# bssrdf/CUDA-Winograd

Hardware: AMD Instinct MI355X
Metric: effective_tflops_conv3x3_256_bn_relu_14x14_N128_fp32 (higher is better)
Workload: dtype f32

## Files before the change

### cuda-winograd_amd/csrc/wino_f2_fused_kernel.h

```cpp
#pragma once
#include "wino_common.h"

#include <type_traits>

namespace wino {
namespace fused {

constexpr int TB = 64;
constexpr int KB = 64;
constexpr int BC = 8;
constexpr int NTHREADS = 512;
constexpr int RAW_BYTES = TB * 16 * BC * 4;
constexpr int U_BYTES = 16 * KB * BC * 4;
constexpr int N_RSTAGE = 2, N_USTAGE = 3;
constexpr int LDS_BYTES = N_RSTAGE * RAW_BYTES + N_USTAGE * U_BYTES;
constexpr int U_CHUNK_FLOATS = 16 * KB * BC;
constexpr int PF = 2;
constexpr int SLAB_BYTES = TB * 4 * KB * 4;
constexpr int DMA0 = 4;

__device__ __forceinline__ void wait_lds(int n) {
  switch (n) {
    case 0: __builtin_amdgcn_s_waitcnt(0xC07F); break;
    case 1: __builtin_amdgcn_s_waitcnt(0xC17F); break;
    case 2: __builtin_amdgcn_s_waitcnt(0xC27F); break;
    case 3: __builtin_amdgcn_s_waitcnt(0xC37F); break;
    case 4: __builtin_amdgcn_s_waitcnt(0xC47F); break;
    case 5: __builtin_amdgcn_s_waitcnt(0xC57F); break;
    case 6: __builtin_amdgcn_s_waitcnt(0xC67F); break;
    case 7: __builtin_amdgcn_s_waitcnt(0xC77F); break;
    case 8: __builtin_amdgcn_s_waitcnt(0xC87F); break;
    case 9: __builtin_amdgcn_s_waitcnt(0xC97F); break;
    case 10: __builtin_amdgcn_s_waitcnt(0xCA7F); break;
    case 11: __builtin_amdgcn_s_waitcnt(0xCB7F); break;
    case 12: __builtin_amdgcn_s_waitcnt(0xCC7F); break;
    default: __builtin_amdgcn_s_waitcnt(0xCF7F); break;
  }
}
constexpr int lds_nr(int q) { return q < 6 ? 2 : 0; }
constexpr int lds_n(int q) { return 2 + lds_nr(q); }
constexpr int lds_wait_count(int e) {
  int after = 15;
  if (e >= PF) {
    after = lds_nr(e - PF);
    for (int q = e - PF + 1; q <= e; q++) after += lds_n(q);
  }
  return after > 15 ? 15 : after;
}

__device__ __forceinline__ f32x2 lds_read2(int addr) {
  return *(const __attribute__((address_space(3))) f32x2*)(size_t)(unsigned)addr;
}
struct TileCoord {
  int n, ty, tx;
};
__device__ __forceinline__ TileCoord decode_tile(int g) {
  TileCoord t;
  t.n = g / WINO_TILES;
  const int rem = g - t.n * WINO_TILES;
  t.ty = rem / 7;
  t.tx = rem - t.ty * 7;
  return t;
}

struct Geo {
  int Hp, Wp;
  unsigned tiles, tiles_x;
  FastDiv d_tiles, d_tx;
};
template <bool GEN>
__device__ __forceinline__ TileCoord decode_tile_g(int g, const Geo& geo) {
  if (!GEN) return decode_tile(g);
  TileCoord t;
  t.n = (int)fastdiv((unsigned)g, geo.d_tiles);
  const unsigned rem = (unsigned)g - (unsigned)t.n * geo.tiles;
  t.ty = (int)fastdiv(rem, geo.d_tx);
  t.tx = (int)(rem - (unsigned)t.ty * geo.tiles_x);
  return t;
}

__host__ __device__ inline unsigned sk_start(unsigned l, unsigned q, unsigned rem, unsigned G) {
  return l * q + l * rem / G;
}

__host__ __device__ inline int tail_range_of(int j, int P, int inv, int copies) {
  const int r = j / copies, b = j - r * copies;
  return (inv * r) % P + P * b;
}
__device__ __forceinline__ int tail_range_of_fast(int j, int P, int inv, int copies, FastDiv d_P, FastDiv d_copies) {
  const int r = (int)fastdiv((unsigned)j, d_copies), b = j - r * copies;
  const int ir = inv * r;
  return ir - (int)fastdiv((unsigned)ir, d_P) * P + P * b;
}

struct FusedParams {
  const float* in;
  const float* Uq;
  int N, C, K, relu, nTB;
  int ndp;
  unsigned sk_q, sk_rem;
  int kp;
  int Gp;
  int ph_P, ph_inv, ph_copies;
  FastDiv d_kp, d_P, d_copies;
  Geo geo;
  const float* bnBias;
  const float* bnScale;
  float* out;
  float* slabs;
  unsigned* tickets;
  unsigned* err;
  unsigned long long* dbg;
};
struct FusedResParams : FusedParams {
  const float* res;
};
template <bool RES>
using FusedArgs = std::conditional_t<RES, FusedResParams, FusedParams>;
constexpr int EPI_PLAIN = 0, EPI_RES = 1, EPI_POOL = 2;

inline void fused_work_layout(FusedParams& p, long long items, int G) {
  const int nchunks = p.C / BC, kblk = p.K / KB;
  const int kp = kblk <= 1 || (G % kblk) != 0 ? 1 : kblk;
  const long long Tg = (items % G) * nchunks / kp, Gp = G / kp, q = Tg / Gp, rem = Tg % Gp;
  p.ndp = (int)(items / G);
  p.sk_q = (unsigned)q;
  p.sk_rem = (unsigned)rem;
  p.kp = kp;
  p.Gp = (int)Gp;
  p.ph_P = 1, p.ph_inv = 0, p.ph_copies = (int)Gp;
  if (rem == 0 && q > 0) {
    long long a = q % nchunks, b = nchunks;
    while (a) { const long long t = b % a; b = a; a = t; }
    const long long g = b, P = nchunks / g;
    if (P > 1 && Gp % P == 0) {
      const long long qq = (q / g) % P;
      for (long long x = 1; x < P; x++)
        if ((qq * x) % P == 1) { p.ph_P = (int)P; p.ph_inv = (int)x; p.ph_copies = (int)(Gp / P); break; }
    }
  }
  p.d_kp = make_fastdiv((unsigned)kp);
  p.d_P = make_fastdiv((unsigned)p.ph_P);
  p.d_copies = make_fastdiv((unsigned)p.ph_copies);
}

__device__ unsigned long long wino_clk_slot_3x3[4];

template <int ABLATE, bool GEN = false, bool TAIL = true, int EPI = EPI_PLAIN>
__global__ void __launch_bounds__(NTHREADS, 2)
wino_f2_fused_kernel(const FusedArgs<EPI == EPI_RES> prm) {
  static_assert(EPI == EPI_PLAIN || EPI == EPI_RES || EPI == EPI_POOL, "epilogue form");
  constexpr bool RES = EPI == EPI_RES, POOL = EPI == EPI_POOL;
  extern __shared__ __attribute__((aligned(16))) char smem[];
  const float* in = prm.in;
  const float* Uq = prm.Uq;
  asm volatile("" : "+s"(in), "+s"(Uq));
  const int N = prm.N, C = prm.C, K = prm.K;
  const unsigned sk_q = prm.sk_q, sk_rem = prm.sk_rem;
  const int ndp = prm.ndp;

  const int KBLK = K >> 6;
  const int nchunks = C / BC;
  const int G = gridDim.x;
  const int lg = (int)(blockIdx.x & 7) * (G >> 3) + ((int)(blockIdx.x & 7) < (G & 7) ? (int)(blockIdx.x & 7) : (G & 7)) +
                 (int)(blockIdx.x >> 3);
  if (ABLATE & PROBE_TIMELINE) {
    if (threadIdx.x == 0) {
      prm.dbg[(size_t)lg * TL_WORDS + TL_ENTRY] = __builtin_amdgcn_s_memrealtime();
      prm.dbg[(size_t)lg * TL_WORDS + TL3_ENTRY_CYC] = __builtin_amdgcn_s_memtime();
    }
  }
  if (ABLATE == PROBE_OFF && blockIdx.x == 0 && threadIdx.x == 0) {
    wino_clk_slot_3x3[0] = __builtin_amdgcn_s_memtime();
    wino_clk_slot_3x3[1] = __builtin_amdgcn_s_memrealtime();
  }
  auto clk_exit = [&]() {
    if (ABLATE == PROBE_OFF && blockIdx.x == 0 && threadIdx.x == 0) {
      wino_clk_slot_3x3[2] = __builtin_amdgcn_s_memtime();
      wino_clk_slot_3x3[3] = __builtin_amdgcn_s_memrealtime();
    }
  };
  const int tail_item0 = ndp * G;
  const int kpg = prm.kp, Gp = prm.Gp;
  const int lpos = __builtin_amdgcn_readfirstlane((int)fastdiv((unsigned)lg, prm.d_kp)), grp = lg - lpos * kpg;
  const int lp = __builtin_amdgcn_readfirstlane(tail_range_of_fast(lpos, prm.ph_P, prm.ph_inv, prm.ph_copies, prm.d_P, prm.d_copies));
  const unsigned t_begin = __builtin_amdgcn_readfirstlane(sk_start(lp, sk_q, sk_rem, Gp));
  const int Lt = (int)(__builtin_amdgcn_readfirstlane(sk_start(lp + 1, sk_q, sk_rem, Gp)) - t_begin);
  const int L = Lt + ndp * nchunks;

  auto ring_pass = [&]() {
    if (ABLATE & PROBE_NO_STORE) return;
    const unsigned Hi = GEN ? (unsigned)prm.geo.Hp : (unsigned)WINO_HW, Wi = GEN ? (unsigned)prm.geo.Wp : (unsigned)WINO_HW;
    const unsigned Hp = POOL ? (Hi - 2u) / 2u + 2u : Hi, Wp = POOL ? (Wi - 2u) / 2u + 2u : Wi;
    const unsigned rpx = 2u * Wp + 2u * (Hp - 2u);
    const unsigned upp = (unsigned)K >> 2;
    const unsigned long long U = (unsigned long long)N * rpx * upp;
    const unsigned u_begin = (unsigned)(U * (unsigned)lg / (unsigned)G);
    const unsigned u_end = (unsigned)(U * ((unsigned)lg + 1u) / (unsigned)G);
    const auto rsrc_ring = make_rsrc(prm.out, (unsigned)((size_t)N * Hp * Wp * K * sizeof(float)));
    const f32x4 zero4 = {0.f, 0.f, 0.f, 0.f};
    for (unsigned u = u_begin + threadIdx.x; u < u_end; u += NTHREADS) {
      const unsigned pid = u / upp, unit = u - pid * upp;
      const unsigned n = pid / rpx, q = pid - n * rpx;
      const unsigned y = q < Wp ? 0u : q < 2 * Wp ? Hp - 1 : q < 2 * Wp + Hp - 2 ? q - 2 * Wp + 1 : q - 2 * Wp - (Hp - 2) + 1;
      const unsigned x = q < Wp ? q : q < 2 * Wp ? q - Wp : q < 2 * Wp + Hp - 2 ? 0u : Wp - 1;
      buf_store16(zero4, rsrc_ring, (((n * Hp + y) * Wp + x) * (unsigned)K + unit * 4u) * (unsigned)sizeof(float), 0);
    }
  };
  if (L <= 0) {
    ring_pass();
    clk_exit();
    return;
  }

  const int tid = threadIdx.x;
  const int lane = tid & 63;
  const int w = __builtin_amdgcn_readfirstlane(tid >> 6);
  const int wt = w >> 1;
  const int ph = w & 1;

  const unsigned u_off = lane * 16;
  const unsigned u_chunk_stride = (unsigned)(KBLK * U_CHUNK_FLOATS * sizeof(float));
  const auto rsrc_in = make_rsrc(in, (unsigned)((size_t)N * (GEN ? prm.geo.Hp * prm.geo.Wp : WINO_HW * WINO_HW) * C * sizeof(float)));
  const auto rsrc_u = make_rsrc(Uq, (unsigned)((size_t)16 * C * K * sizeof(float)));

  const int t16 = lane & 15, h = lane >> 4;
  const int lds0 = (int)(unsigned)(size_t)(__attribute__((address_space(3))) char*)smem;
  const int a_base = lds0 + (wt * 16 + t16) * 512 + ((h ^ (((t16 >> 3) & 1) << 1)) << 3);
  const int a_sw = t16 & 7;
  int a_adr[3][4];
#pragma unroll
  for (int k = 0; k < 3; k++) {
    const int row = ph ? (k == 0 ? 2 : k == 1 ? 1 : 3) : (k == 0 ? 0 : k == 1 ? 2 : 1);
#pragma unroll
    for (int j = 0; j < 4; j++) {
      const int px = 4 * row + j;
      a_adr[k][j] = a_base + (((px & 7) ^ a_sw) << 5) + ((px >> 3) << 8);
    }
  }
  int b_base[4];
#pragma unroll
  for (int cb = 0; cb < 4; cb++) {
    const int kl = (cb ^ (2 * ph)) * 16 + t16;
    b_base[cb] = lds0 + N_RSTAGE * RAW_BYTES + ph * (8 * 2048) + kl * 32 + ((h ^ (((kl >> 3) & 1) << 1)) << 3);
  }
  asm volatile("" : "+v"(b_base[1]), "+v"(b_base[2]), "+v"(b_base[3]));

  typedef f32x2 P2;
  auto sub2 = [](const P2& a, const P2& b) { return a - b; };
  auto add2 = [](const P2& a, const P2& b) { return a + b; };
  const float s2f = ph ? -1.f : 1.f;
  const P2 s2 = {s2f, s2f};
  auto tmp_col = [&](P2* tmp, const P2* d, int j) {
    tmp[0 * 4 + j] = sub2(d[0 * 4 + j], d[1 * 4 + j]);
    tmp[1 * 4 + j] = d[1 * 4 + j] + s2 * d[2 * 4 + j];
  };
  auto v_point = [&](P2* v, const P2* tmp, int e) {
    const int i = e >> 2, j = e & 3;
    if (j == 0) v[e] = sub2(tmp[i * 4 + 0], tmp[i * 4 + 2]);
    if (j == 1) v[e] = add2(tmp[i * 4 + 1], tmp[i * 4 + 2]);
    if (j == 2) v[e] = sub2(tmp[i * 4 + 2], tmp[i * 4 + 1]);
    if (j == 3) v[e] = sub2(tmp[i * 4 + 1], tmp[i * 4 + 3]);
  };

  unsigned long long st_wait = 0, st_comp = 0, st_epi = 0, st_prev = 0;
  unsigned long long st_ph[4] = {0, 0, 0, 0};
  auto stamp = [&]() -> unsigned long long {
    unsigned long long t;
    __builtin_amdgcn_sched_barrier(0);
    asm volatile("s_memtime %0\n\ts_waitcnt lgkmcnt(0)" : "=s"(t)::"memory");
    __builtin_amdgcn_sched_barrier(0);
    return t;
  };

  typedef const __attribute__((address_space(4))) FusedParams* KernargPtr;
  auto kernarg = []() {
    KernargPtr kp = (KernargPtr)__builtin_amdgcn_kernarg_segment_ptr();
    asm volatile("" : "+s"(kp));
    return kp;
  };
  auto load_geo = [](KernargPtr kp) {
    Geo g;
    g.Hp = kp->geo.Hp; g.Wp = kp->geo.Wp; g.tiles = kp->geo.tiles; g.tiles_x = kp->geo.tiles_x;
    g.d_tiles.m = kp->geo.d_tiles.m; g.d_tiles.l = kp->geo.d_tiles.l;
    g.d_tx.m = kp->geo.d_tx.m; g.d_tx.l = kp->geo.d_tx.l;
    return g;
  };

  unsigned raw_off[4];
  unsigned d_soff_raw = 0;
  unsigned d_soff_u = 0;
  int d_item, d_chunk, d_tail, d_tb = -1;
  auto dma_set_item = [&](int item) {
    const int tb = item / KBLK, kb = item - tb * KBLK;
    d_item = item;
    if (tb != d_tb) {
      d_tb = tb;
      KernargPtr kp = kernarg();
      const Geo geo = load_geo(kp);
      const int Wp = GEN ? geo.Wp : WINO_HW, Hp = GEN ? geo.Hp : WINO_HW;
      const int C = kp->C, totalTiles = kp->N * (GEN ? (int)geo.tiles : WINO_TILES);
      const int up = lane & 31;
      const int pxp = up >> 1, halfp = up & 1;
#pragma unroll
      for (int j = 0; j < 4; j++) {
        const int tl = 16 * j + 2 * w + (lane >> 5);
        const int px = pxp ^ (tl & 7);
        const int half = halfp ^ ((tl >> 3) & 1);
        int g = tb * TB + tl;
        g = g < totalTiles ? g : totalTiles - 1;
        const TileCoord tc = decode_tile_g<GEN>(g, geo);
        const int y = 2 * tc.ty + (px >> 2), x = 2 * tc.tx + (px & 3);
        raw_off[j] = (unsigned)((((size_t)(tc.n * Hp + y) * Wp + x) * C + half * 4) * sizeof(float));
      }
    }
    d_soff_raw = __builtin_amdgcn_readfirstlane((unsigned)(d_chunk * (BC * sizeof(float))));
    d_soff_u = __builtin_amdgcn_readfirstlane((unsigned)((kb * U_CHUNK_FLOATS + w * 256) * sizeof(float)) + d_chunk * u_chunk_stride);
    asm volatile("" : "+s"(d_soff_raw), "+s"(d_soff_u));
  };
  auto pin_dma_state = [&]() {
    d_item = __builtin_amdgcn_readfirstlane(d_item);
    d_chunk = __builtin_amdgcn_readfirstlane(d_chunk);
    d_tail = __builtin_amdgcn_readfirstlane(d_tail);
    d_tb = __builtin_amdgcn_readfirstlane(d_tb);
    asm volatile("" : "+s"(d_item), "+s"(d_chunk), "+s"(d_tail), "+s"(d_tb));
  };
  auto dma_advance = [&]() {
    if (d_tail > 0 && --d_tail == 0) {
      d_chunk = 0;
      dma_set_item(lg);
    } else if (++d_chunk == nchunks) {
      d_chunk = 0;
      dma_set_item(d_tail > 0 ? d_item + kernarg()->kp : d_item + G);
    } else {
      d_soff_raw += (unsigned)(BC * sizeof(float));
      d_soff_u += u_chunk_stride;
      asm volatile("" : "+s"(d_soff_raw), "+s"(d_soff_u));
    }
    pin_dma_state();
  };
  auto issue_raw1 = [&](int rstage, int j) {
    if (ABLATE & PROBE_NO_DMA_A) return;
    dma16_buf(rsrc_in, raw_off[j], d_soff_raw, smem + rstage * RAW_BYTES + (8 * j + w) * 1024);
  };
  auto issue_u1 = [&](int ustage, int j) {
    if (ABLATE & PROBE_NO_DMA_B) return;
    dma16_buf(rsrc_u, u_off, d_soff_u + j * 8192,
              smem + N_RSTAGE * RAW_BYTES + ustage * U_BYTES + (8 * j + w) * 1024);
  };

  int c_tail_vg = Lt;
  int c_item_vg = __builtin_amdgcn_readfirstlane(Lt > 0 ? tail_item0 + (int)(t_begin / (unsigned)nchunks) * kpg + grp : lg);
  int c_chunk = __builtin_amdgcn_readfirstlane(Lt > 0 ? (int)(t_begin % (unsigned)nchunks) : 0);
  int seg_kind_vg = 0;
  int pend_vg = -1;
  asm volatile("" : "+v"(pend_vg));

  f32x4 acc[8][4];
#pragma unroll
  for (int e = 0; e < 8; e++)
#pragma unroll
    for (int cb = 0; cb < 4; cb++) acc[e][cb] = (f32x4){0.f, 0.f, 0.f, 0.f};
  P2 v[8];
  f32x2 bfn[PF][2];

  d_chunk = c_chunk;
  d_tail = Lt;
  dma_set_item(c_item_vg);
  asm volatile("" : "+v"(c_item_vg));
#pragma unroll
  for (int j = 0; j < 4; j++) issue_raw1(0, j);
#pragma unroll
  for (int j = 0; j < 4; j++) issue_u1(0, j);
  if ((ABLATE & PROBE_TIMELINE) && tid == 0) prm.dbg[(size_t)lg * TL_WORDS + TL3_STAGE_REQ] = __builtin_amdgcn_s_memrealtime();
  if (L > 1) dma_advance();
  ring_pass();
  if (!(ABLATE & PROBE_NO_SYNC)) {
    wait_vmem_all();
    __syncthreads();
  }
  if ((ABLATE & PROBE_TIMELINE) && tid == 0) prm.dbg[(size_t)lg * TL_WORDS + TL3_STAGE_IN] = __builtin_amdgcn_s_memrealtime();
  if (L > 1) {
#pragma unroll
    for (int j = 0; j < 4; j++) issue_raw1(1, j);
#pragma unroll
    for (int j = 0; j < 4; j++) issue_u1(1, j);
    if (L > 2) dma_advance();
  }
  {
    P2 d[12];
#pragma unroll
    for (int k = 0; k < 3; k++)
#pragma unroll
      for (int j = 0; j < 4; j++) d[k * 4 + j] = lds_read2(a_adr[k][j]);
    P2 tmp[8];
#pragma unroll
    for (int j = 0; j < 4; j++) tmp_col(tmp, d, j);
#pragma unroll
    for (int e = 0; e < 8; e++) v_point(v, tmp, e);
#pragma unroll
    for (int e = 0; e < PF; e++) {
      bfn[e][0] = lds_read2(b_base[2 * (e & 1) + 0] + (e >> 1) * 2048);
      bfn[e][1] = lds_read2(b_base[2 * (e & 1) + 1] + (e >> 1) * 2048);
    }
  }
  if (ABLATE & PROBE_TIMELINE) {
    if (tid == 0) prm.dbg[(size_t)lg * TL_WORDS + TL_FIRST] = __builtin_amdgcn_s_memrealtime();
  }
  if (ABLATE & PROBE_CLOCK) {
    if (tid == 0) {
      prm.dbg[(size_t)lg * CLK_WORDS + CLK_BEGIN_CYC] = __builtin_amdgcn_s_memtime();
      prm.dbg[(size_t)lg * CLK_WORDS + CLK_BEGIN_RT] = __builtin_amdgcn_s_memrealtime();
    }
  }

  int ub_cur[4], ub_nxt[4];
#pragma unroll
  for (int cb = 0; cb < 4; cb++) {
    ub_cur[cb] = b_base[cb];
    ub_nxt[cb] = b_base[cb] + U_BYTES;
  }
  auto body = [&](auto par_c, int it, int rs_dma, int us_dma) {
    constexpr int ROFF = decltype(par_c)::value ? 0 : RAW_BYTES;
    if (ABLATE & PROBE_PHASES) { const unsigned long long t = stamp(); if (it) st_comp += t - st_prev; st_prev = t; }
    if (!(ABLATE & PROBE_NO_SYNC)) {
      wait_vmem_all();
      __syncthreads();
    }
    if (ABLATE & PROBE_PHASES) { const unsigned long long t = stamp(); st_wait += t - st_prev; st_prev = t; }
    const int (&ucur)[4] = decltype(par_c)::value ? ub_nxt : ub_cur;
    const int (&unxt)[4] = decltype(par_c)::value ? ub_cur : ub_nxt;
    auto bread = [&](const int (&base)[4], int s2_, int c) {
      return lds_read2(base[2 * (s2_ & 1) + c] + (s2_ >> 1) * 2048);
    };

    f32x2 bf[16][2];
#pragma unroll
    for (int e = 0; e < PF; e++) { bf[e][0] = bfn[e][0]; bf[e][1] = bfn[e][1]; }
    P2 d[12], tmp[8];
    __builtin_amdgcn_sched_barrier(0);
#pragma unroll
    for (int e = 0; e < 16; e++) {
      const int pt = e >> 1, cbp = e & 1;
      if (ABLATE & PROBE_NO_B_READS) {
        const f32x2 fake = {v[(e + 3) & 7].x, v[(e + 5) & 7].y};
        if (e + PF < 16) { bf[e + PF][0] = fake; bf[e + PF][1] = fake; }
        else { bfn[e + PF - 16][0] = fake; bfn[e + PF - 16][1] = fake; }
      } else if (e + PF < 16) {
        bf[e + PF][0] = bread(ucur, e + PF, 0);
        bf[e + PF][1] = bread(ucur, e + PF, 1);
      } else {
        bfn[e + PF - 16][0] = bread(unxt, e + PF - 16, 0);
        bfn[e + PF - 16][1] = bread(unxt, e + PF - 16, 1);
      }
      if (e >= DMA0 && e < DMA0 + 4) {
        issue_raw1(rs_dma, e - DMA0);
      } else if (e >= DMA0 + 4 && e < DMA0 + 8) {
        issue_u1(us_dma, e - DMA0 - 4);
      }
      if (e < 6 && !(ABLATE & PROBE_NO_A_PATH)) {
        const int q0 = 2 * e, q1 = 2 * e + 1;
        d[(q0 % 3) * 4 + q0 / 3] = lds_read2(a_adr[q0 % 3][q0 / 3] + ROFF);
        d[(q1 % 3) * 4 + q1 / 3] = lds_read2(a_adr[q1 % 3][q1 / 3] + ROFF);
      }
      __builtin_amdgcn_sched_barrier(0);
      if (!(ABLATE & (PROBE_NO_A_PATH | PROBE_NO_B_READS))) wait_lds(lds_wait_count(e));
      __builtin_amdgcn_sched_barrier(0);
      if (e >= 3 && e <= 7 && e != 5 && !(ABLATE & PROBE_NO_A_PATH) && !(ABLATE & PROBE_NO_BTDB)) tmp_col(tmp, d, e == 3 ? 0 : e == 4 ? 1 : e == 6 ? 2 : 3);
      if ((ABLATE & PROBE_NO_BTDB) && e == 7) {
#pragma unroll
        for (int i = 0; i < 12; i++) asm volatile("" :: "v"(d[i]));
      }
      const P2 a = v[pt];
      const f32x2 b0 = bf[e][0], b1 = bf[e][1];
      if (ABLATE & PROBE_NO_MFMA) {
        asm volatile("" ::"v"(a.x), "v"(a.y), "v"(b0.x), "v"(b0.y), "v"(b1.x), "v"(b1.y));
      } else {
        asm volatile("v_mfma_f32_16x16x4_f32 %0, %1, %2, %0" : "+v"(acc[pt][2 * cbp + 0]) : "v"(a.x), "v"(b0.x));
        asm volatile("v_mfma_f32_16x16x4_f32 %0, %1, %2, %0" : "+v"(acc[pt][2 * cbp + 1]) : "v"(a.x), "v"(b1.x));
        asm volatile("v_mfma_f32_16x16x4_f32 %0, %1, %2, %0" : "+v"(acc[pt][2 * cbp + 0]) : "v"(a.y), "v"(b0.y));
        asm volatile("v_mfma_f32_16x16x4_f32 %0, %1, %2, %0" : "+v"(acc[pt][2 * cbp + 1]) : "v"(a.y), "v"(b1.y));
      }
      if ((ABLATE & PROBE_NO_VPOINT) && !(ABLATE & PROBE_NO_BTDB) && e == 9) {
#pragma unroll
        for (int i = 0; i < 8; i++) asm volatile("" :: "v"(tmp[i]));
      }
      if (!(ABLATE & PROBE_NO_A_PATH) && !(ABLATE & (PROBE_NO_VPOINT | PROBE_NO_BTDB))) {
        if (e >= 9 && e < 15) v_point(v, tmp, e - 9);
        if (e == 15) {
          v_point(v, tmp, 6);
          v_point(v, tmp, 7);
        }
      }
      __builtin_amdgcn_sched_barrier(0);
    }
  };

  auto epilogue = [&](bool last_of_range, int rfree, int ufree) {
    unsigned long long ph_t = 0;
    auto phase = [&](int k) { if (ABLATE & PROBE_PHASES) { const unsigned long long t = stamp(); if (k >= 0) st_ph[k] += t - ph_t; ph_t = t; } };
    phase(-1);
    asm volatile("" ::: "memory");
    __builtin_amdgcn_s_barrier();
    asm volatile("s_nop 15\n\ts_nop 15" ::: "memory");
    phase(0);
    int ln = lane, wv = w;
    asm volatile("" : "+v"(ln));
    asm volatile("" : "+s"(wv));
    const int e_t16 = ln & 15, e_h = ln >> 4, e_wt = wv >> 1, e_wk = wv & 1;
    char* wreg = smem + (wv < 4 ? rfree + wv * 8192 : ufree + (wv - 4) * 8192);
    KernargPtr kp = kernarg();
    const Geo geo = load_geo(kp);
    const int Wp = GEN ? geo.Wp : WINO_HW, Hp = GEN ? geo.Hp : WINO_HW;
    const int N = kp->N, K = kp->K, relu = kp->relu, KBLK = K >> 6, totalTiles = N * (GEN ? (int)geo.tiles : WINO_TILES);
    const unsigned sk_q = kp->sk_q, sk_rem = kp->sk_rem;
    const int tail_item0 = kp->ndp * G;
    struct TailPos { int kpg, Gp, lp, grp; FastDiv d_kp; };
    auto tail_pos = [&]() {
      TailPos t;
      t.kpg = kp->kp; t.Gp = kp->Gp;
      t.d_kp.m = kp->d_kp.m; t.d_kp.l = kp->d_kp.l;
      FastDiv dP, dC;
      dP.m = kp->d_P.m; dP.l = kp->d_P.l; dC.m = kp->d_copies.m; dC.l = kp->d_copies.l;
      const int lpos_e = (int)fastdiv((unsigned)lg, t.d_kp);
      t.grp = lg - lpos_e * t.kpg;
      t.lp = tail_range_of_fast(lpos_e, kp->ph_P, kp->ph_inv, kp->ph_copies, dP, dC);
      return t;
    };
    const float* bnBias = kp->bnBias;
    const float* bnScale = kp->bnScale;
    unsigned* tickets = kp->tickets;
    const int Hq = POOL ? (Hp - 2) / 2 + 2 : Hp, Wq = POOL ? (Wp - 2) / 2 + 2 : Wp;
    const auto rsrc_out = make_rsrc(kp->out, (unsigned)((size_t)N * Hq * Wq * K * sizeof(float)));
    const auto rsrc_slab = make_rsrc(kp->slabs, (unsigned)((size_t)2 * G * SLAB_BYTES));
    const unsigned slab_voff = (unsigned)((wv * 8 * 64 + ln) * 16);

    auto load_bn = [&](int item, float (&sc)[2], float (&bi)[2]) {
      const int kb = item % KBLK;
#pragma unroll
      for (int cb = 0; cb < 2; cb++) {
        const int kc = kb * KB + e_wk * 32 + cb * 16 + e_t16;
        sc[cb] = bnScale[kc];
        bi[cb] = bnBias[kc];
      }
    };
    auto draw_ticket = [&](int item) -> unsigned {
      unsigned old = 0;
      if (ln == 0)
        old = __hip_atomic_fetch_add(tickets + (size_t)item * 8 + wv, 1u, __ATOMIC_RELAXED, __HIP_MEMORY_SCOPE_AGENT);
      return old;
    };

    const int c_item = __builtin_amdgcn_readfirstlane(c_item_vg), seg_kind = __builtin_amdgcn_readfirstlane(seg_kind_vg);
    float bn_sc[2], bn_bi[2];
    load_bn(c_item, bn_sc, bn_bi);
    int pend_item = __builtin_amdgcn_readfirstlane(pend_vg);
    unsigned pend_old = 0;
    if (TAIL && pend_item >= 0) pend_old = draw_ticket(pend_item);
    const bool ph1 = (wv & 1) != 0;
    auto part = [&](int r, int cb) {
      float c[2][2];
#pragma unroll
      for (int i = 0; i < 2; i++) {
        const float m0 = acc[i * 4 + 0][cb][r], m1 = acc[i * 4 + 1][cb][r];
        const float m2 = acc[i * 4 + 2][cb][r], m3 = acc[i * 4 + 3][cb][r];
        c[i][0] = m0 + m1 + m2;
        c[i][1] = m1 - m2 - m3;
      }
      f32x4 o;
#pragma unroll
      for (int bb = 0; bb < 2; bb++) {
        const float sum = c[0][bb] + c[1][bb];
        o[bb] = ph1 ? c[0][bb] : sum;
        o[2 + bb] = ph1 ? -sum : c[1][bb];
      }
      return o;
    };
    f32x4 y[4][2];
    {
      char* const xmine = wreg + ln * 16;
      const char* const xpart = smem + ((wv ^ 1) < 4 ? rfree + (wv ^ 1) * 8192 : ufree + ((wv ^ 1) - 4) * 8192) + ln * 16;
#pragma unroll
      for (int r = 0; r < 4; r++)
#pragma unroll
        for (int cb = 0; cb < 2; cb++) *(f32x4*)(xmine + (2 * r + cb) * 1024) = part(r, 2 + cb);
#pragma unroll
      for (int r = 0; r < 4; r++)
#pragma unroll
        for (int cb = 0; cb < 2; cb++) y[r][cb] = part(r, cb);
      asm volatile("s_waitcnt lgkmcnt(0)" ::: "memory");
      __builtin_amdgcn_s_barrier();
      asm volatile("" ::: "memory");
#pragma unroll
      for (int r = 0; r < 4; r++)
#pragma unroll
        for (int cb = 0; cb < 2; cb++) y[r][cb] += *(const f32x4*)(xpart + (2 * r + cb) * 1024);
      asm volatile("s_waitcnt lgkmcnt(0)" ::: "memory");
      __builtin_amdgcn_s_barrier();
      asm volatile("" ::: "memory");
    }
#pragma unroll
    for (int e = 0; e < 8; e++)
#pragma unroll
      for (int cb = 0; cb < 4; cb++) acc[e][cb] = (f32x4){0.f, 0.f, 0.f, 0.f};
    phase(1);
    const bool whole = !TAIL || (seg_kind & 1) != 0;
    int job0 = -1, job1 = TAIL ? pend_item : -1;
    pend_item = -1;
    unsigned old0 = 0;
    if (whole) {
      job0 = c_item;
    } else if (!(ABLATE & PROBE_NO_HANDOFF)) {
      const TailPos tp = tail_pos();
      const unsigned my_slot = 2u * (unsigned)(tp.lp * tp.kpg + tp.grp) + ((seg_kind & 2) ? 1u : 0u);
#pragma unroll
      for (int q = 0; q < 8; q++)
        slab_store16(y[q >> 1][q & 1], rsrc_slab, slab_voff + q * 1024, my_slot * SLAB_BYTES);
      const bool now = last_of_range || ((seg_kind & 2) && job1 >= 0);
      if (!now) {
        pend_item = c_item;
      } else {
        wait_vmem_all();
        old0 = draw_ticket(c_item);
        job0 = c_item;
      }
    }
    pend_vg = pend_item;
    asm volatile("" : "+v"(pend_vg));
    phase(2);
#pragma unroll 1
    for (int j = 0; j < (TAIL ? 2 : 1); j++) {
      const int item = j == 0 ? job0 : job1;
      if (item < 0) continue;
      if (!(j == 0 && whole)) {
        const TailPos tp = tail_pos();
        const int kpg = tp.kpg, Gp = tp.Gp, grp_e = tp.grp;
        const unsigned x0 = fastdiv((unsigned)(item - tail_item0), tp.d_kp) * (unsigned)nchunks, x1 = x0 + nchunks - 1;
        int gA = tp.lp, gB = tp.lp;
        while (sk_start(gA, sk_q, sk_rem, Gp) > x0) gA--;
        while (gB + 1 < Gp && sk_start(gB + 1, sk_q, sk_rem, Gp) <= x1) gB++;
        int nseg = 0;
        for (int g = gA; g <= gB; g++)
          nseg += sk_start(g + 1, sk_q, sk_rem, Gp) != sk_start(g, sk_q, sk_rem, Gp);
        const unsigned old = __builtin_amdgcn_readfirstlane(j == 0 ? old0 : pend_old);
        if (old != (unsigned)(nseg - 1)) {
          if (old >= (unsigned)nseg && ln == 0) __hip_atomic_store(kp->err, 1u, __ATOMIC_RELAXED, __HIP_MEMORY_SCOPE_SYSTEM);
          continue;
        }
        if (ln == 0)
          __hip_atomic_fetch_sub(tickets + (size_t)item * 8 + wv, (unsigned)nseg, __ATOMIC_RELAXED, __HIP_MEMORY_SCOPE_AGENT);
        bool first = true;
#pragma unroll 1
        for (int g = gA; g <= gB; g++) {
          if (sk_start(g + 1, sk_q, sk_rem, Gp) == sk_start(g, sk_q, sk_rem, Gp)) continue;
          const unsigned slot = 2u * (unsigned)(g * kpg + grp_e) + (first ? 1u : 0u);
          f32x4 t[8];
#pragma unroll
          for (int q = 0; q < 8; q++) t[q] = slab_load16(rsrc_slab, slab_voff + q * 1024, slot * SLAB_BYTES);
#pragma unroll
          for (int q = 0; q < 8; q++) y[q >> 1][q & 1] = first ? t[q] : y[q >> 1][q & 1] + t[q];
          first = false;
        }
      }
      float sc2[2] = {bn_sc[0], bn_sc[1]}, bi2[2] = {bn_bi[0], bn_bi[1]};
      if (item != c_item) load_bn(item, sc2, bi2);
      if (ABLATE & PROBE_NO_STORE) continue;

      const int tb = item / KBLK, kb = item - tb * KBLK;
      f32x4 rv[RES ? 8 : 1];
      if constexpr (RES) {
        typedef const __attribute__((address_space(4))) FusedResParams* ResKernargPtr;
        const auto rsrc_res = make_rsrc(((ResKernargPtr)kp)->res, (unsigned)((size_t)N * Hp * Wp * K * sizeof(float)));
        const int px = (ln >> 3) & 3, pa = px >> 1, pb = px & 1;
        const unsigned kbyte = (unsigned)((kb * KB + e_wk * 32 + (ln & 7) * 4) * sizeof(float));
#pragma unroll
        for (int i = 0; i < 8; i++) {
          const int g = tb * TB + e_wt * 16 + 2 * i + (ln >> 5);
          const bool live = g < totalTiles;
          const TileCoord tc = decode_tile_g<GEN>(live ? g : 0, geo);
          const int py = 1 + 2 * tc.ty + pa, pxx = 1 + 2 * tc.tx + pb;
          const unsigned img = (unsigned)(tc.n * Hp * Wp);
          rv[i] = (f32x4){0.f, 0.f, 0.f, 0.f};
          if (live && (!GEN || (py <= Hp - 2 && pxx <= Wp - 2)))
            rv[i] = buf_load16(rsrc_res, (unsigned)((img + py * Wp + pxx) * K * sizeof(float)) + kbyte, 0);
        }
      }
      if constexpr (POOL) {
#pragma unroll
        for (int r = 0; r < 4; r++) {
#pragma unroll
          for (int cb = 0; cb < 2; cb++) {
            float m = 0.f;
#pragma unroll
            for (int pp = 0; pp < 4; pp++) {
              float v1 = sc2[cb] * y[r][cb][pp] + bi2[cb];
              if (relu) v1 = relu_nan(v1);
              m = pp == 0 ? v1 : max_nan(m, v1);
            }
            *(float*)(wreg + (4 * r + e_h) * 128 + ((cb ^ (e_h >> 1)) << 6) + e_t16 * 4) = m;
          }
        }
        const unsigned kbyte = (unsigned)((kb * KB + e_wk * 32 + (ln & 7) * 4) * sizeof(float));
#pragma unroll
        for (int i = 0; i < 2; i++) {
          const int P = 8 * i + (ln >> 3), ph_t = P & 3, tl = 4 * ph_t + (P >> 2);
          const f32x4 val = *(const f32x4*)(wreg + P * 128 + (((((ln & 7) >> 2) ^ (ph_t >> 1))) << 6) + (ln & 3) * 16);
          const int g = tb * TB + e_wt * 16 + tl;
          const bool live = g < totalTiles;
          const TileCoord tc = decode_tile_g<GEN>(live ? g : 0, geo);
          const int py = 1 + tc.ty, pxx = 1 + tc.tx;
          const unsigned img = (unsigned)(tc.n * Hq * Wq);
          const bool keep = live && (!GEN || (py <= Hq - 2 && pxx <= Wq - 2));
          if (keep) buf_store16_nt(val, rsrc_out, (unsigned)((img + py * Wq + pxx) * K * sizeof(float)) + kbyte, 0);
        }
        continue;
      }
      int ep_wbase[4], ep_rbase[4];
#pragma unroll
      for (int jj = 0; jj < 4; jj++) {
        ep_wbase[jj] = e_h * 2048 + ((jj ^ e_h) << 6) + e_t16 * 4;
        const int px = (ln >> 3) & 3, c = ln & 7;
        ep_rbase[jj] = (ln >> 5) * 512 + (((px * 2 + (c >> 2)) ^ jj) << 6) + (c & 3) * 16;
      }
#pragma unroll
      for (int r = 0; r < 4; r++) {
#pragma unroll
        for (int cb = 0; cb < 2; cb++) {
#pragma unroll
          for (int pp = 0; pp < 4; pp++) {
            float v1 = sc2[cb] * y[r][cb][pp] + bi2[cb];
            if (!RES && relu) v1 = relu_nan(v1);
            const int g = pp * 2 + cb;
            *(float*)(wreg + ep_wbase[g & 3] + r * 512 + (g >> 2) * 256) = v1;
          }
        }
      }
      const int px = (ln >> 3) & 3, pa = px >> 1, pb = px & 1;
      const unsigned kbyte = (unsigned)((kb * KB + e_wk * 32 + (ln & 7) * 4) * sizeof(float));
#pragma unroll
      for (int i = 0; i < 8; i++) {
        f32x4 val = *(const f32x4*)(wreg + ep_rbase[i >> 1] + i * 1024);
        if constexpr (RES) {
          val += rv[i];
          if (relu) {
#pragma unroll
            for (int q = 0; q < 4; q++) val[q] = relu_nan(val[q]);
          }
        }
        const int g = tb * TB + e_wt * 16 + 2 * i + (ln >> 5);
        const bool live = g < totalTiles;
        const TileCoord tc = decode_tile_g<GEN>(live ? g : 0, geo);
        const int py = 1 + 2 * tc.ty + pa, pxx = 1 + 2 * tc.tx + pb;
        const unsigned img = (unsigned)(tc.n * Hp * Wp);
        const bool keep = live && (!GEN || (py <= Hp - 2 && pxx <= Wp - 2));
        if (keep) buf_store16_nt(val, rsrc_out, (unsigned)((img + py * Wp + pxx) * K * sizeof(float)) + kbyte, 0);
      }
    }
    phase(3);
  };

  {
    int us = 0;
    auto next = [](int s) { return s == 2 ? 0 : s + 1; };
    int it = 0;
#pragma unroll 1
    for (;;) {
      int c_tail = __builtin_amdgcn_readfirstlane(c_tail_vg);
      const int n = c_tail > 0 && c_tail < nchunks - c_chunk ? c_tail : nchunks - c_chunk;
      seg_kind_vg = c_chunk == 0 ? (n == nchunks ? 3 : 2) : 0;
      asm volatile("" : "+v"(seg_kind_vg));
      if (c_tail > 0 && (c_tail -= n) == 0) c_tail = -1;
      c_tail_vg = c_tail;
      asm volatile("" : "+v"(c_tail_vg));
      c_chunk = 0;
      int us_last = us;
      auto tail = [&](auto par_c) {
        if (it + 3 < L) dma_advance();
        us_last = us;
        us = next(us);
        it++;
        {
          const int off = next(us) * U_BYTES;
#pragma unroll
          for (int cb = 0; cb < 4; cb++) {
            if (decltype(par_c)::value) ub_nxt[cb] = b_base[cb] + off;
            else ub_cur[cb] = b_base[cb] + off;
          }
        }
      };
      {
        int k = n;
#pragma unroll 1
        for (;;) {
          if (!(it & 1)) {
            body(std::integral_constant<int, 0>{}, it, 0, next(next(us)));
            tail(std::integral_constant<int, 0>{});
            if (--k == 0) break;
          }
          body(std::integral_constant<int, 1>{}, it, 1, next(next(us)));
          tail(std::integral_constant<int, 1>{});
          if (--k == 0) break;
        }
      }
      const bool last_of_range = it == L;
      if (ABLATE & PROBE_PHASES) { const unsigned long long t = stamp(); st_comp += t - st_prev; st_prev = t; }
      if ((ABLATE & PROBE_TIMELINE) && last_of_range && tid == 0) {
        KernargPtr kp = kernarg();
        kp->dbg[(size_t)lg * TL_WORDS + TL_LAST_EPI] = __builtin_amdgcn_s_memrealtime();
      }
      epilogue(last_of_range, (it & 1) * RAW_BYTES, N_RSTAGE * RAW_BYTES + us_last * U_BYTES);
      if (ABLATE & PROBE_PHASES) { const unsigned long long t = stamp(); st_epi += t - st_prev; st_prev = t; }
      if (last_of_range) break;
      c_tail = __builtin_amdgcn_readfirstlane(c_tail_vg);
      if (c_tail < 0) {
        c_item_vg = lg;
        c_tail_vg = 0;
      } else {
        c_item_vg += c_tail > 0 ? kernarg()->kp : G;
      }
      asm volatile("" : "+v"(c_item_vg), "+v"(c_tail_vg));
    }
  }
  wait_vmem_all();
  clk_exit();

  if (ABLATE & PROBE_PHASES) {
    if (lane == 0) {
      unsigned long long* dbg = prm.dbg + ((size_t)lg * PH_WAVES + w) * PH_WORDS;
      dbg[PH_WAIT] = st_wait;
      dbg[PH_COMPUTE] = st_comp;
      dbg[PH_EPILOGUE] = st_epi;
      dbg[PH_EPI0 + 0] = st_ph[0];
      dbg[PH_EPI0 + 1] = st_ph[1];
      dbg[PH_EPI0 + 2] = st_ph[2];
      dbg[PH_EPI0 + 3] = st_ph[3];
    }
  }
  if (ABLATE & PROBE_TIMELINE) {
    if (tid == 0) {
      KernargPtr kp = kernarg();
      kp->dbg[(size_t)lg * TL_WORDS + TL_EXIT] = __builtin_amdgcn_s_memrealtime();
      kp->dbg[(size_t)lg * TL_WORDS + TL3_EXIT_CYC] = __builtin_amdgcn_s_memtime();
    }
  }
  if (ABLATE & PROBE_CLOCK) {
    if (tid == 0) {
      KernargPtr kp = kernarg();
      unsigned long long* dbg = kp->dbg + (size_t)lg * CLK_WORDS;
      dbg[CLK_END_CYC] = __builtin_amdgcn_s_memtime();
      dbg[CLK_END_RT] = __builtin_amdgcn_s_memrealtime();
    }
  }
}

}
}
```

### cuda-winograd_amd/csrc/wino_probe.h

```cpp
#pragma once

namespace wino {

constexpr int PROBE_OFF = 0, PROBE_NO_DMA_A = 1, PROBE_NO_DMA_B = 2, PROBE_NO_MFMA = 4, PROBE_NO_SYNC = 8,
              PROBE_CLOCK = 16, PROBE_NO_A_PATH = 32, PROBE_NO_B_READS = 64, PROBE_NO_STORE = 512,
              PROBE_NO_HANDOFF = 1024, PROBE_PHASES = 2048, PROBE_NO_VPOINT = 4096, PROBE_NO_BTDB = 8192,
              PROBE_TIMELINE = 32768;

constexpr int TL_WORDS = 8, TL_ENTRY = 0, TL_FIRST = 1, TL_LAST_EPI = 2, TL_EXIT = 3;
constexpr int TL3_ENTRY_CYC = 4, TL3_EXIT_CYC = 5, TL3_STAGE_REQ = 6, TL3_STAGE_IN = 7;
constexpr int TL1_HW_ID = 4, TL1_ENTRY_CYC = 5, TL1_EXIT_CYC = 6;
constexpr int CLK_WORDS = 4, CLK_BEGIN_CYC = 0, CLK_BEGIN_RT = 1, CLK_END_CYC = 2, CLK_END_RT = 3;
constexpr int PH_WORDS = 8, PH_WAVES = 8, PH_USED = 7, PH_WAIT = 0, PH_COMPUTE = 1, PH_EPILOGUE = 2, PH_EPI0 = 3;
constexpr int SM_WORDS = 8, SM_ENTRY = 0, SM_STAGED = 1, SM_MFMA_DONE = 2, SM_LDS_LEVEL = 3, SM_SLAB_OUT = 4,
              SM_TICKET = 5, SM_GATHERED = 6, SM_EXIT = 7;

}
```

Before: 248.2.

## Restructure DMA/compute loop into run-length segments with lane-spilled scalar state

Replaces the per-iteration DMA advance branching with precomputed run lengths: the inner loop now only adds fixed offsets, and item/chunk transitions are handled as rare events between runs. Scheduler state that was held in scalar registers is moved into lanes of a VGPR via writelane/readlane to relieve SGPR pressure. The B^T d B transform is moved out of the interleaved MFMA schedule to the end of the body. A span timing probe is also added. The aim is to cut scalar control overhead in the hot loop, at the cost of more complex bookkeeping and the loss of overlap between the transform and the MFMAs.

```diff
diff --git a/cuda-winograd_amd/csrc/wino_f2_fused_kernel.h b/cuda-winograd_amd/csrc/wino_f2_fused_kernel.h
--- a/cuda-winograd_amd/csrc/wino_f2_fused_kernel.h
+++ b/cuda-winograd_amd/csrc/wino_f2_fused_kernel.h
@@ -263,7 +263,7 @@
     if (j == 3) v[e] = sub2(tmp[i * 4 + 1], tmp[i * 4 + 3]);
   };
 
-  unsigned long long st_wait = 0, st_comp = 0, st_epi = 0, st_prev = 0;
+  unsigned long long st_wait = 0, st_comp = 0, st_epi = 0, st_prev = 0, st_span = 0;
   unsigned long long st_ph[4] = {0, 0, 0, 0};
   auto stamp = [&]() -> unsigned long long {
     unsigned long long t;
@@ -290,12 +290,21 @@
   unsigned raw_off[4];
   unsigned d_soff_raw = 0;
   unsigned d_soff_u = 0;
-  int d_item, d_chunk, d_tail, d_tb = -1;
-  auto dma_set_item = [&](int item) {
+  unsigned d_step_raw = (unsigned)(BC * sizeof(float)), d_step_u = u_chunk_stride;
+  int d_run = 0;
+  int ws_vg = 0;
+  typedef std::integral_constant<int, 0> WS_D_ITEM; typedef std::integral_constant<int, 1> WS_D_TAIL;
+  typedef std::integral_constant<int, 2> WS_D_LEFT; typedef std::integral_constant<int, 3> WS_D_TB;
+  typedef std::integral_constant<int, 4> WS_D_RUN;  typedef std::integral_constant<int, 5> WS_C_RUN;
+  typedef std::integral_constant<int, 6> WS_C_LEFT;
+  auto ws_put = [&ws_vg](auto slot, int val) { asm volatile("v_writelane_b32 %0, %1, %2" : "+v"(ws_vg) : "s"(val), "n"(decltype(slot)::value)); };
+  auto ws_get = [&ws_vg](auto slot) { return __builtin_amdgcn_readlane(ws_vg, decltype(slot)::value); };
+  ws_put(WS_D_TB{}, -1);
+  constexpr int D_NEVER = 0x7fffffff;
+  auto dma_set_item = [&](int item, int chunk) {
     const int tb = item / KBLK, kb = item - tb * KBLK;
-    d_item = item;
-    if (tb != d_tb) {
-      d_tb = tb;
+    if (tb != ws_get(WS_D_TB{})) {
+      ws_put(WS_D_TB{}, tb);
       KernargPtr kp = kernarg();
       const Geo geo = load_geo(kp);
       const int Wp = GEN ? geo.Wp : WINO_HW, Hp = GEN ? geo.Hp : WINO_HW;
@@ -314,29 +323,51 @@
         raw_off[j] = (unsigned)((((size_t)(tc.n * Hp + y) * Wp + x) * C + half * 4) * sizeof(float));
       }
     }
-    d_soff_raw = __builtin_amdgcn_readfirstlane((unsigned)(d_chunk * (BC * sizeof(float))));
-    d_soff_u = __builtin_amdgcn_readfirstlane((unsigned)((kb * U_CHUNK_FLOATS + w * 256) * sizeof(float)) + d_chunk * u_chunk_stride);
-    asm volatile("" : "+s"(d_soff_raw), "+s"(d_soff_u));
+    asm volatile("" : "+v"(raw_off[0]), "+v"(raw_off[1]), "+v"(raw_off[2]), "+v"(raw_off[3]));
+    d_soff_raw = __builtin_amdgcn_readfirstlane((unsigned)(chunk * (BC * sizeof(float))));
+    d_soff_u = __builtin_amdgcn_readfirstlane((unsigned)((kb * U_CHUNK_FLOATS + w * 256) * sizeof(float)) + chunk * u_chunk_stride);
   };
   auto pin_dma_state = [&]() {
-    d_item = __builtin_amdgcn_readfirstlane(d_item);
-    d_chunk = __builtin_amdgcn_readfirstlane(d_chunk);
-    d_tail = __builtin_amdgcn_readfirstlane(d_tail);
-    d_tb = __builtin_amdgcn_readfirstlane(d_tb);
-    asm volatile("" : "+s"(d_item), "+s"(d_chunk), "+s"(d_tail), "+s"(d_tb));
+    d_run = __builtin_amdgcn_readfirstlane(d_run);
+    asm volatile("" : "+s"(d_soff_raw), "+s"(d_soff_u), "+s"(d_step_raw), "+s"(d_step_u), "+s"(d_run));
+  };
+  auto dma_stand = [&]() {
+    d_step_raw = 0;
+    d_step_u = 0;
+    d_run = D_NEVER;
+  };
+  auto dma_plan = [&](int item, int chunk, int tail, int left) {
+    const int nch = kernarg()->C / BC;
+    const int in_item = nch - 1 - chunk;
+    const int plain = tail > 0 && tail - 1 < in_item ? tail - 1 : in_item;
+    if (left <= plain) {
+      if (left == 0) dma_stand();
+      else d_run = left;
+      left = -1;
+    } else {
+      d_run = plain + 1;
+      left -= plain + 1;
+      if (tail > 0) tail -= plain;
+    }
+    ws_put(WS_D_ITEM{}, item), ws_put(WS_D_TAIL{}, tail), ws_put(WS_D_LEFT{}, left);
+  };
+  auto dma_event = [&]() {
+    int item = ws_get(WS_D_ITEM{}), tail = ws_get(WS_D_TAIL{});
+    const int left = ws_get(WS_D_LEFT{});
+    if (left < 0) {
+      dma_stand();
+    } else {
+      if (tail > 0 && --tail == 0) item = lg;
+      else item += tail > 0 ? kernarg()->kp : G;
+      dma_set_item(item, 0);
+      dma_plan(item, 0, tail, left);
+    }
+    pin_dma_state();
   };
   auto dma_advance = [&]() {
-    if (d_tail > 0 && --d_tail == 0) {
-      d_chunk = 0;
-      dma_set_item(lg);
-    } else if (++d_chunk == nchunks) {
-      d_chunk = 0;
-      dma_set_item(d_tail > 0 ? d_item + kernarg()->kp : d_item + G);
-    } else {
-      d_soff_raw += (unsigned)(BC * sizeof(float));
-      d_soff_u += u_chunk_stride;
-      asm volatile("" : "+s"(d_soff_raw), "+s"(d_soff_u));
-    }
+    d_soff_raw += d_step_raw;
+    d_soff_u += d_step_u;
+    if (--d_run == 0) dma_event();
     pin_dma_state();
   };
   auto issue_raw1 = [&](int rstage, int j) {
@@ -364,16 +395,16 @@
   P2 v[8];
   f32x2 bfn[PF][2];
 
-  d_chunk = c_chunk;
-  d_tail = Lt;
-  dma_set_item(c_item_vg);
+  dma_set_item(c_item_vg, c_chunk);
+  dma_plan(c_item_vg, c_chunk, Lt, L - 1);
+  pin_dma_state();
   asm volatile("" : "+v"(c_item_vg));
 #pragma unroll
   for (int j = 0; j < 4; j++) issue_raw1(0, j);
 #pragma unroll
   for (int j = 0; j < 4; j++) issue_u1(0, j);
   if ((ABLATE & PROBE_TIMELINE) && tid == 0) prm.dbg[(size_t)lg * TL_WORDS + TL3_STAGE_REQ] = __builtin_amdgcn_s_memrealtime();
-  if (L > 1) dma_advance();
+  dma_advance();
   ring_pass();
   if (!(ABLATE & PROBE_NO_SYNC)) {
     wait_vmem_all();
@@ -385,7 +416,7 @@
     for (int j = 0; j < 4; j++) issue_raw1(1, j);
 #pragma unroll
     for (int j = 0; j < 4; j++) issue_u1(1, j);
-    if (L > 2) dma_advance();
+    dma_advance();
   }
   {
     P2 d[12];
@@ -420,9 +451,9 @@
     ub_cur[cb] = b_base[cb];
     ub_nxt[cb] = b_base[cb] + U_BYTES;
   }
-  auto body = [&](auto par_c, int it, int rs_dma, int us_dma) {
+  auto body = [&](auto par_c, int rs_dma, int us_dma) {
     constexpr int ROFF = decltype(par_c)::value ? 0 : RAW_BYTES;
-    if (ABLATE & PROBE_PHASES) { const unsigned long long t = stamp(); if (it) st_comp += t - st_prev; st_prev = t; }
+    if (ABLATE & PROBE_PHASES) { const unsigned long long t = stamp(); if (st_prev) st_comp += t - st_prev; st_prev = t; }
     if (!(ABLATE & PROBE_NO_SYNC)) {
       wait_vmem_all();
       __syncthreads();
@@ -466,11 +497,6 @@
       __builtin_amdgcn_sched_barrier(0);
       if (!(ABLATE & (PROBE_NO_A_PATH | PROBE_NO_B_READS))) wait_lds(lds_wait_count(e));
       __builtin_amdgcn_sched_barrier(0);
-      if (e >= 3 && e <= 7 && e != 5 && !(ABLATE & PROBE_NO_A_PATH) && !(ABLATE & PROBE_NO_BTDB)) tmp_col(tmp, d, e == 3 ? 0 : e == 4 ? 1 : e == 6 ? 2 : 3);
-      if ((ABLATE & PROBE_NO_BTDB) && e == 7) {
-#pragma unroll
-        for (int i = 0; i < 12; i++) asm volatile("" :: "v"(d[i]));
-      }
       const P2 a = v[pt];
       const f32x2 b0 = bf[e][0], b1 = bf[e][1];
       if (ABLATE & PROBE_NO_MFMA) {
@@ -481,18 +507,24 @@
         asm volatile("v_mfma_f32_16x16x4_f32 %0, %1, %2, %0" : "+v"(acc[pt][2 * cbp + 0]) : "v"(a.y), "v"(b0.y));
         asm volatile("v_mfma_f32_16x16x4_f32 %0, %1, %2, %0" : "+v"(acc[pt][2 * cbp + 1]) : "v"(a.y), "v"(b1.y));
       }
-      if ((ABLATE & PROBE_NO_VPOINT) && !(ABLATE & PROBE_NO_BTDB) && e == 9) {
-#pragma unroll
-        for (int i = 0; i < 8; i++) asm volatile("" :: "v"(tmp[i]));
-      }
-      if (!(ABLATE & PROBE_NO_A_PATH) && !(ABLATE & (PROBE_NO_VPOINT | PROBE_NO_BTDB))) {
-        if (e >= 9 && e < 15) v_point(v, tmp, e - 9);
-        if (e == 15) {
-          v_point(v, tmp, 6);
-          v_point(v, tmp, 7);
+      if ((ABLATE & PROBE_PHASES) && e == 15) st_span += stamp() - st_prev;
+      __builtin_amdgcn_sched_barrier(0);
+    }
+    if (!(ABLATE & PROBE_NO_A_PATH)) {
+      if (ABLATE & PROBE_NO_BTDB) {
+#pragma unroll
+        for (int i = 0; i < 12; i++) asm volatile("" :: "v"(d[i]));
+      } else {
+#pragma unroll
+        for (int j = 0; j < 4; j++) tmp_col(tmp, d, j);
+        if (ABLATE & PROBE_NO_VPOINT) {
+#pragma unroll
+          for (int i = 0; i < 8; i++) asm volatile("" :: "v"(tmp[i]));
+        } else {
+#pragma unroll
+          for (int e = 0; e < 8; e++) v_point(v, tmp, e);
         }
       }
-      __builtin_amdgcn_sched_barrier(0);
     }
   };
 
@@ -761,57 +793,77 @@
 
   {
     int us = 0;
+    int par = 0;
     auto next = [](int s) { return s == 2 ? 0 : s + 1; };
-    int it = 0;
-#pragma unroll 1
-    for (;;) {
+    int c_run = 0;
+    ws_put(WS_C_LEFT{}, L);
+    auto segment = [&]() {
       int c_tail = __builtin_amdgcn_readfirstlane(c_tail_vg);
       const int n = c_tail > 0 && c_tail < nchunks - c_chunk ? c_tail : nchunks - c_chunk;
       seg_kind_vg = c_chunk == 0 ? (n == nchunks ? 3 : 2) : 0;
       asm volatile("" : "+v"(seg_kind_vg));
       if (c_tail > 0 && (c_tail -= n) == 0) c_tail = -1;
       c_tail_vg = c_tail;
+      ws_put(WS_C_LEFT{}, ws_get(WS_C_LEFT{}) - n);
       asm volatile("" : "+v"(c_tail_vg));
       c_chunk = 0;
-      int us_last = us;
-      auto tail = [&](auto par_c) {
-        if (it + 3 < L) dma_advance();
-        us_last = us;
-        us = next(us);
-        it++;
-        {
-          const int off = next(us) * U_BYTES;
-#pragma unroll
-          for (int cb = 0; cb < 4; cb++) {
-            if (decltype(par_c)::value) ub_nxt[cb] = b_base[cb] + off;
-            else ub_cur[cb] = b_base[cb] + off;
+      c_run = n;
+    };
+    auto tail = [&](auto par_c) {
+      d_soff_raw += d_step_raw;
+      d_soff_u += d_step_u;
+      asm volatile("" : "+s"(d_soff_raw), "+s"(d_soff_u));
+      us = next(us);
+      {
+        const int off = next(us) * U_BYTES;
+#pragma unroll
+        for (int cb = 0; cb < 4; cb++) {
+          if (decltype(par_c)::value) ub_nxt[cb] = b_base[cb] + off;
+          else ub_cur[cb] = b_base[cb] + off;
+        }
+      }
+    };
+    segment();
+#pragma unroll 1
+    for (;;) {
+      {
+        int k = d_run < c_run ? d_run : c_run;
+        ws_put(WS_D_RUN{}, d_run - k), ws_put(WS_C_RUN{}, c_run - k);
+        int skip0 = par;
+        par ^= k & 1;
+#pragma unroll 1
+        do {
+          asm volatile("" : "+s"(skip0));
+          if (!skip0) {
+            body(std::integral_constant<int, 0>{}, 0, next(next(us)));
+            tail(std::integral_constant<int, 0>{});
+            --k;
           }
-        }
-      };
-      {
-        int k = n;
-#pragma unroll 1
-        for (;;) {
-          if (!(it & 1)) {
-            body(std::integral_constant<int, 0>{}, it, 0, next(next(us)));
-            tail(std::integral_constant<int, 0>{});
-            if (--k == 0) break;
+          skip0 = 0;
+          asm volatile("" : "+s"(k));
+          if (k != 0) {
+            body(std::integral_constant<int, 1>{}, 1, next(next(us)));
+            tail(std::integral_constant<int, 1>{});
+            --k;
           }
-          body(std::integral_constant<int, 1>{}, it, 1, next(next(us)));
-          tail(std::integral_constant<int, 1>{});
-          if (--k == 0) break;
-        }
-      }
-      const bool last_of_range = it == L;
+          asm volatile("" : "+s"(k));
+        } while (k != 0);
+        d_run = ws_get(WS_D_RUN{});
+        c_run = ws_get(WS_C_RUN{});
+      }
+      if (d_run == 0) dma_event();
+      if (c_run != 0) continue;
+      const int us_last = us == 0 ? 2 : us - 1;
+      const bool last_of_range = ws_get(WS_C_LEFT{}) == 0;
       if (ABLATE & PROBE_PHASES) { const unsigned long long t = stamp(); st_comp += t - st_prev; st_prev = t; }
       if ((ABLATE & PROBE_TIMELINE) && last_of_range && tid == 0) {
         KernargPtr kp = kernarg();
         kp->dbg[(size_t)lg * TL_WORDS + TL_LAST_EPI] = __builtin_amdgcn_s_memrealtime();
       }
-      epilogue(last_of_range, (it & 1) * RAW_BYTES, N_RSTAGE * RAW_BYTES + us_last * U_BYTES);
+      epilogue(last_of_range, par * RAW_BYTES, N_RSTAGE * RAW_BYTES + us_last * U_BYTES);
       if (ABLATE & PROBE_PHASES) { const unsigned long long t = stamp(); st_epi += t - st_prev; st_prev = t; }
       if (last_of_range) break;
-      c_tail = __builtin_amdgcn_readfirstlane(c_tail_vg);
+      const int c_tail = __builtin_amdgcn_readfirstlane(c_tail_vg);
       if (c_tail < 0) {
         c_item_vg = lg;
         c_tail_vg = 0;
@@ -819,6 +871,7 @@
         c_item_vg += c_tail > 0 ? kernarg()->kp : G;
       }
       asm volatile("" : "+v"(c_item_vg), "+v"(c_tail_vg));
+      segment();
     }
   }
   wait_vmem_all();
@@ -834,6 +887,7 @@
       dbg[PH_EPI0 + 1] = st_ph[1];
       dbg[PH_EPI0 + 2] = st_ph[2];
       dbg[PH_EPI0 + 3] = st_ph[3];
+      dbg[PH_SPAN] = st_span;
     }
   }
   if (ABLATE & PROBE_TIMELINE) {
diff --git a/cuda-winograd_amd/csrc/wino_probe.h b/cuda-winograd_amd/csrc/wino_probe.h
--- a/cuda-winograd_amd/csrc/wino_probe.h
+++ b/cuda-winograd_amd/csrc/wino_probe.h
@@ -11,7 +11,7 @@
 constexpr int TL3_ENTRY_CYC = 4, TL3_EXIT_CYC = 5, TL3_STAGE_REQ = 6, TL3_STAGE_IN = 7;
 constexpr int TL1_HW_ID = 4, TL1_ENTRY_CYC = 5, TL1_EXIT_CYC = 6;
 constexpr int CLK_WORDS = 4, CLK_BEGIN_CYC = 0, CLK_BEGIN_RT = 1, CLK_END_CYC = 2, CLK_END_RT = 3;
-constexpr int PH_WORDS = 8, PH_WAVES = 8, PH_USED = 7, PH_WAIT = 0, PH_COMPUTE = 1, PH_EPILOGUE = 2, PH_EPI0 = 3;
+constexpr int PH_WORDS = 8, PH_WAVES = 8, PH_USED = 8, PH_WAIT = 0, PH_COMPUTE = 1, PH_EPILOGUE = 2, PH_EPI0 = 3, PH_SPAN = 7;
 constexpr int SM_WORDS = 8, SM_ENTRY = 0, SM_STAGED = 1, SM_MFMA_DONE = 2, SM_LDS_LEVEL = 3, SM_SLAB_OUT = 4,
               SM_TICKET = 5, SM_GATHERED = 6, SM_EXIT = 7;
 
```

Result: faster. 252.5, median of 6 (+1.7%).
